# Open-Finance-Lab/RLSolver

Measured on AMD Instinct MI355X. Metric: env-steps/sec (all instances) on Gset G22 MaxCut; achieved HBM GB/s % peak, higher is better.
Workload: dtype u8

## Files before the change

rlsolver_amd/csrc/rls_step.hip:

```cpp
#include "rls_tile.h"
#include <cstdlib>

namespace rls {

constexpr int kStepPad = 128;

template <typename T> __device__ __forceinline__ T spin_flip(T v);
template <> __device__ __forceinline__ uint8_t spin_flip<uint8_t>(uint8_t v) { return v == 0 ? 1 : 0; }
template <> __device__ __forceinline__ float spin_flip<float>(float v) { return v == 0.0f ? 1.0f : 0.0f; }

template <typename T, bool WEIGHTED>
__device__ __forceinline__ int flip_gain(const T* row, int64_t a, const int32_t* __restrict__ rowptr,
                                         const int32_t* __restrict__ col, const int32_t* __restrict__ wgt,
                                         int lane) {
    const int r0 = rowptr[a], r1 = rowptr[a + 1];
    const bool xa = spin_is_set(row[a]);
    int acc = 0;
    for (int j = r0 + lane; j < r1; j += kWave) {
        const bool xn = spin_is_set(row[col[j]]);
        if constexpr (WEIGHTED) acc += (xn == xa) ? wgt[j] : -wgt[j];
        else acc += (xn != xa) ? 1 : 0;
    }
    if constexpr (WEIGHTED) {
        return wave_sum_i32(acc);
    } else {
        int c;
        if (r1 - r0 <= kWave) c = __popcll(ballot64(acc != 0));
        else c = wave_sum_i32(acc);
        return (r1 - r0) - 2 * c;
    }
}

template <bool NT, typename V> __device__ __forceinline__ V ld_vec(const V* p) {
    if constexpr (NT) return __builtin_nontemporal_load(p);
    else return *p;
}
enum : int { kStPlain = 0, kStNt = 1, kStWt = 2 };
template <int ST, typename V> __device__ __forceinline__ void st_vec(V* p, V v) {
    if constexpr (ST == kStNt) {
        __builtin_nontemporal_store(v, p);
    } else if constexpr (ST == kStWt) {
        static_assert(sizeof(V) == 16, "write-through stores are 16-byte vectors");
        asm volatile("global_store_dwordx4 %0, %1, off sc1\n\ts_nop 1" :: "v"(p), "v"(v) : "memory");
    } else {
        *p = v;
    }
}

__device__ __forceinline__ void wait_vmcnt_le(int k) {
    k = __builtin_amdgcn_readfirstlane(k);
#define RLS_W(n) case n: asm volatile("s_waitcnt vmcnt(" #n ")" ::: "memory"); break;
#define RLS_W8(b) RLS_W(b + 0) RLS_W(b + 1) RLS_W(b + 2) RLS_W(b + 3) RLS_W(b + 4) RLS_W(b + 5) RLS_W(b + 6) RLS_W(b + 7)
    switch (k) {
        case 0: asm volatile("s_waitcnt vmcnt(0)" ::: "memory"); break;
        RLS_W(1) RLS_W(2) RLS_W(3) RLS_W(4) RLS_W(5) RLS_W(6) RLS_W(7)
        RLS_W(8) RLS_W(9) RLS_W(10) RLS_W(11) RLS_W(12) RLS_W(13) RLS_W(14) RLS_W(15)
        RLS_W(16) RLS_W(17) RLS_W(18) RLS_W(19) RLS_W(20) RLS_W(21) RLS_W(22) RLS_W(23)
        RLS_W(24) RLS_W(25) RLS_W(26) RLS_W(27) RLS_W(28) RLS_W(29) RLS_W(30) RLS_W(31)
        RLS_W(32) RLS_W(33) RLS_W(34) RLS_W(35) RLS_W(36) RLS_W(37) RLS_W(38) RLS_W(39)
        RLS_W(40) RLS_W(41) RLS_W(42) RLS_W(43) RLS_W(44) RLS_W(45) RLS_W(46) RLS_W(47)
        RLS_W(48) RLS_W(49) RLS_W(50) RLS_W(51) RLS_W(52) RLS_W(53) RLS_W(54) RLS_W(55)
        RLS_W(56) RLS_W(57) RLS_W(58) RLS_W(59) RLS_W(60) RLS_W(61) RLS_W(62)
        default: asm volatile("s_waitcnt vmcnt(63)" ::: "memory"); break;
    }
#undef RLS_W8
#undef RLS_W
}

template <typename T, int EPW, int MODE, bool EMIT, bool VEC, bool WEIGHTED, bool NTL, int ST>
__global__ __launch_bounds__(256) void k_maxcut_step(const T* __restrict__ xin, T* __restrict__ xout,
                                                     int64_t B, int64_t N,
                                                     const int32_t* __restrict__ rowptr,
                                                     const int32_t* __restrict__ col,
                                                     const int32_t* __restrict__ wgt,
                                                     const int64_t* __restrict__ action,
                                                     int32_t* __restrict__ obj, float* __restrict__ reward,
                                                     float* __restrict__ cur, float* __restrict__ done,
                                                     float done_value, int align_lines) {
    extern __shared__ __attribute__((aligned(16))) unsigned char smem[];
    const int lane = threadIdx.x & (kWave - 1);
    const int wib = __builtin_amdgcn_readfirstlane((int)(threadIdx.x / kWave));
    using V = typename SpinVec<T>::type;
    constexpr int PER = SpinVec<T>::n;
    const int64_t wave_stride = (int64_t)gridDim.x * (blockDim.x / kWave);
  for (int64_t wave = (int64_t)blockIdx.x * (blockDim.x / kWave) + wib; wave * EPW < B; wave += wave_stride) {
    const int64_t b0 = wave * EPW;
    const int nenv = (int)((B - b0) < EPW ? (B - b0) : EPW);

    int64_t act[EPW];
#pragma unroll
    for (int k = 0; k < EPW; ++k) {
        const int64_t a = (k < nenv) ? action[b0 + k] : -1;
        act[k] = ((uint64_t)a < (uint64_t)N) ? a : -1;
    }

    int my_delta = 0;
    auto publish = [&]() {
        if (lane < nenv) {
            const int64_t b = b0 + lane;
            bool ok = false;
#pragma unroll
            for (int k = 0; k < EPW; ++k) if (lane == k) ok = act[k] >= 0;
            const int v = obj[b] + my_delta;
            obj[b] = v;
            reward[b] = ok ? (float)my_delta : __builtin_nanf("");
            if (cur) cur[b] = (float)v;
            if (done) done[b] = done_value;
        }
    };

    if constexpr (!EMIT) {
#pragma unroll
        for (int k = 0; k < EPW; ++k)
            if (act[k] >= 0) {
                const int d = flip_gain<T, WEIGHTED>(xin + (b0 + k) * N, act[k], rowptr, col, wgt, lane);
                if (lane == k) my_delta = d;
            }
        publish();
        if (lane < nenv) {
            int64_t a = -1;
#pragma unroll
            for (int k = 0; k < EPW; ++k) if (lane == k) a = act[k];
            if (a >= 0) {
                T* p = xout + (b0 + lane) * N + a;
                *p = spin_flip<T>(*p);
            }
        }
        return;
    } else if constexpr (!VEC) {
#pragma unroll
        for (int k = 0; k < EPW; ++k)
            if (act[k] >= 0) {
                const int d = flip_gain<T, WEIGHTED>(xin + (b0 + k) * N, act[k], rowptr, col, wgt, lane);
                if (lane == k) my_delta = d;
            }
        publish();
        const T* src = xin + b0 * N;
        T* dst = xout + b0 * N;
        const int64_t nel = (int64_t)nenv * N;
        for (int64_t i = lane; i < nel; i += kWave) {
            T v = src[i];
#pragma unroll
            for (int k = 0; k < EPW; ++k)
                if (act[k] >= 0 && i == (int64_t)k * N + act[k]) v = spin_flip<T>(v);
            dst[i] = v;
        }
        continue;
    } else {
        const V* src = reinterpret_cast<const V*>(xin + b0 * N);
        V* dst = reinterpret_cast<V*>(xout + b0 * N);
        const int64_t nel = (int64_t)nenv * N;
        const int64_t nvec = nel / PER;
        auto tail_copy = [&]() {
            for (int64_t i = nvec * PER + lane; i < nel; i += kWave) {
                T v = xin[b0 * N + i];
#pragma unroll
                for (int k = 0; k < EPW; ++k)
                    if (act[k] >= 0 && i == (int64_t)k * N + act[k]) v = spin_flip<T>(v);
                xout[b0 * N + i] = v;
            }
        };
        int64_t fvec[EPW];
        int fidx[EPW];
#pragma unroll
        for (int k = 0; k < EPW; ++k) {
            const int64_t rel = (act[k] < 0) ? -1 : (int64_t)k * N + act[k];
            fvec[k] = rel < 0 ? -1 : rel / PER;
            fidx[k] = (int)(rel < 0 ? 0 : rel % PER);
        }

        if constexpr (MODE == 0) {
#pragma unroll
            for (int k = 0; k < EPW; ++k)
                if (act[k] >= 0) {
                    const int d = flip_gain<T, WEIGHTED>(xin + (b0 + k) * N, act[k], rowptr, col, wgt, lane);
                    if (lane == k) my_delta = d;
                }
            publish();
#pragma unroll 4
            for (int64_t i = lane; i < nvec; i += kWave) {
                V v = ld_vec<NTL>(src + i);
#pragma unroll
                for (int k = 0; k < EPW; ++k)
                    if (i == fvec[k]) v = SpinVec<T>::flip_at(v, fidx[k]);
                st_vec<ST>(dst + i, v);
            }
            tail_copy();
        } else if constexpr (MODE == 1) {
            constexpr int BATCH = 8;
            V buf[BATCH];
            bool first = true;
            for (int64_t base = 0; base < nvec; base += BATCH * kWave) {
#pragma unroll
                for (int q = 0; q < BATCH; ++q) {
                    const int64_t i = base + q * kWave + lane;
                    if (i < nvec) buf[q] = ld_vec<NTL>(src + i);
                }
                if (first) {
                    first = false;
#pragma unroll
                    for (int k = 0; k < EPW; ++k)
                        if (act[k] >= 0) {
                            const int d = flip_gain<T, WEIGHTED>(xin + (b0 + k) * N, act[k], rowptr, col, wgt, lane);
                            if (lane == k) my_delta = d;
                        }
                    publish();
                }
#pragma unroll
                for (int q = 0; q < BATCH; ++q) {
                    const int64_t i = base + q * kWave + lane;
                    if (i < nvec) {
                        V v = buf[q];
#pragma unroll
                        for (int k = 0; k < EPW; ++k)
                            if (i == fvec[k]) v = SpinVec<T>::flip_at(v, fidx[k]);
                        st_vec<ST>(dst + i, v);
                    }
                }
            }
            tail_copy();
        } else if constexpr (MODE == 3) {
            unsigned char* region = smem + (size_t)wib * ((size_t)EPW * N * sizeof(T) + kStepPad);
            const int h_in = (int)((reinterpret_cast<uintptr_t>(src) >> 4) & 7), h_out = (int)((reinterpret_cast<uintptr_t>(dst) >> 4) & 7);
            const int h = (align_lines && h_in == h_out) ? h_in : 0;
            V* region_v = reinterpret_cast<V*>(region);
            V* stage_v = region_v + h;
            T* stage = reinterpret_cast<T*>(stage_v);
            const int nch = (int)((nvec + h + kWave - 1) / kWave);
            for (int64_t slot0 = 0; slot0 < nvec + h; slot0 += kWave) {
                const int64_t i = slot0 + lane - h;
                if (i >= 0 && i < nvec) glds16<NTL>(src + i, region_v + slot0);
            }
            if (nvec * PER < nel) {
                for (int64_t i = nvec * PER + lane; i < nel; i += kWave) stage[i] = xin[b0 * N + i];
                asm volatile("s_waitcnt vmcnt(0)" ::: "memory");
            }
            int r0[EPW], deg[EPW], nb[EPW], nlo = 0;
#pragma unroll
            for (int k = 0; k < EPW; ++k) {
                r0[k] = 0; deg[k] = 0; nb[k] = 0;
                if (act[k] >= 0) {
                    r0[k] = rowptr[act[k]];
                    deg[k] = rowptr[act[k] + 1] - r0[k];
                    if (deg[k] > 0) {
                        const int32_t* pn = col + r0[k] + (lane < deg[k] ? lane : 0);
                        asm volatile("global_load_dword %0, %1, off" : "=v"(nb[k]) : "v"(pn) : "memory");
                        ++nlo;
                    }
                }
            }
            const int keep = nch - 1 + nlo;
            for (int j = 0; j < nch; ++j) {
                wait_vmcnt_le(keep);
                const int64_t i = (int64_t)j * kWave + lane - h;
                if (i >= 0 && i < nvec) {
                    V v = stage_v[i];
#pragma unroll
                    for (int k = 0; k < EPW; ++k)
                        if (i == fvec[k]) v = SpinVec<T>::flip_at(v, fidx[k]);
                    st_vec<ST>(dst + i, v);
                }
            }
            tail_copy();
            wait_vmcnt_le(nch < 62 ? nch : 62);
#pragma unroll
            for (int k = 0; k < EPW; ++k) asm volatile("" : "+v"(nb[k]) :: "memory");
#pragma unroll
            for (int k = 0; k < EPW; ++k)
                if (act[k] >= 0) {
                    const T* row = stage + (int64_t)k * N;
                    const bool xa = spin_is_set(row[act[k]]);
                    int d;
                    if (deg[k] <= kWave) {
                        const bool on = lane < deg[k];
                        const bool xn = on ? spin_is_set(row[nb[k]]) : xa;
                        d = deg[k] - 2 * __popcll(ballot64(xn != xa));
                    } else {
                        d = flip_gain<T, WEIGHTED>(row, act[k], rowptr, col, wgt, lane);
                    }
                    if (lane == k) my_delta = d;
                }
            publish();
        } else {
            unsigned char* region = smem + (size_t)wib * ((size_t)EPW * N * sizeof(T) + kStepPad);
            const int h_in = align_lines ? (int)((reinterpret_cast<uintptr_t>(src) >> 4) & 7) : 0;
            const int h_out = align_lines ? (int)((reinterpret_cast<uintptr_t>(dst) >> 4) & 7) : 0;
            V* region_v = reinterpret_cast<V*>(region);
            V* stage_v = region_v + h_in;
            T* stage = reinterpret_cast<T*>(stage_v);
            for (int64_t slot0 = 0; slot0 < nvec + h_in; slot0 += kWave) {
                const int64_t i = slot0 + lane - h_in;
                if (i >= 0 && i < nvec) glds16<NTL>(src + i, region_v + slot0);
            }
            for (int64_t i = nvec * PER + lane; i < nel; i += kWave) stage[i] = xin[b0 * N + i];
            int r0[EPW], deg[EPW], nb[EPW], wv[EPW];
#pragma unroll
            for (int k = 0; k < EPW; ++k) {
                r0[k] = 0; deg[k] = 0; nb[k] = 0; wv[k] = 0;
                if (act[k] >= 0) {
                    r0[k] = rowptr[act[k]];
                    deg[k] = rowptr[act[k] + 1] - r0[k];
                    if (lane < deg[k]) {
                        nb[k] = col[r0[k] + lane];
                        if constexpr (WEIGHTED) wv[k] = wgt[r0[k] + lane];
                    }
                }
            }
            asm volatile("s_waitcnt vmcnt(0) lgkmcnt(0)" ::: "memory");
            __builtin_amdgcn_wave_barrier();
#pragma unroll
            for (int k = 0; k < EPW; ++k)
                if (act[k] >= 0) {
                    const T* row = stage + (int64_t)k * N;
                    const bool xa = spin_is_set(row[act[k]]);
                    int d;
                    if (deg[k] <= kWave) {
                        const bool on = lane < deg[k];
                        const bool xn = on ? spin_is_set(row[nb[k]]) : xa;
                        if constexpr (WEIGHTED) d = wave_sum_i32(on ? ((xn == xa) ? wv[k] : -wv[k]) : 0);
                        else d = deg[k] - 2 * __popcll(ballot64(xn != xa));
                    } else {
                        d = flip_gain<T, WEIGHTED>(row, act[k], rowptr, col, wgt, lane);
                    }
                    if (lane == k) my_delta = d;
                }
            publish();
            __builtin_amdgcn_wave_barrier();
            if (lane < nenv) {
                int64_t a = -1;
#pragma unroll
                for (int k = 0; k < EPW; ++k) if (lane == k) a = act[k];
                if (a >= 0) {
                    T* p = stage + (int64_t)lane * N + a;
                    *p = spin_flip<T>(*p);
                }
            }
            asm volatile("s_waitcnt lgkmcnt(0)" ::: "memory");
            __builtin_amdgcn_wave_barrier();
#pragma unroll 4
            for (int64_t slot0 = 0; slot0 < nvec + h_out; slot0 += kWave) {
                const int64_t i = slot0 + lane - h_out;
                if (i >= 0 && i < nvec) st_vec<ST>(dst + i, stage_v[i]);
            }
            for (int64_t i = nvec * PER + lane; i < nel; i += kWave) xout[b0 * N + i] = stage[i];
        }
    }
  }
}

struct StepKnobs { int nts, epw, wpb, persist, chase, align, wt; };
static StepKnobs step_knobs() {
    return StepKnobs{(int)knob(KN_STEP_NTS, -1), (int)knob(KN_STEP_EPW, 0), (int)knob(KN_STEP_WPB, 0), (int)knob(KN_STEP_PERSIST, -1),
                     (int)knob(KN_STEP_CHASE, -1), (int)knob(KN_STEP_ALIGN, 1), (int)knob(KN_STEP_WT, -1)};
}

}

using namespace rls;

extern "C" int rls_maxcut_step(const rls_graph* g, const void* x_in, void* x_out, int spin_bytes, int64_t B,
                               const int64_t* action, int32_t* obj, float* reward, float* cur, float* done,
                               float done_value, void* stream) {
    if (int rc = check_graph(g)) return rc;
    RLS_REQUIRE(B >= 0, RLS_EINVAL, "B < 0");
    if (B == 0) return RLS_OK;
    RLS_REQUIRE(x_in && x_out && action && obj && reward, RLS_EINVAL, "x_in/x_out/action/obj/reward is NULL");
    RLS_REQUIRE(spin_bytes == 1 || spin_bytes == 4, RLS_EINVAL, "spin_bytes must be 1 or 4");
    RLS_REQUIRE(!g->wgt, RLS_EUNSUPPORTED, "rls_maxcut_step counts cut edges (env_PPO.py:108-121): build the graph without weights");
    const int64_t N = g->num_nodes;
    const bool emit = (x_in != x_out);
    RLS_REQUIRE(!emit || (const char*)x_in + (size_t)B * N * spin_bytes <= (const char*)x_out ||
                    (const char*)x_out + (size_t)B * N * spin_bytes <= (const char*)x_in,
                RLS_EINVAL, "x_in and x_out overlap partially");
    const StepKnobs knobs = step_knobs();
    int epw_auto = 8;
    while (epw_auto > 1 && (int64_t)epw_auto * N * spin_bytes > 8192) epw_auto >>= 1;
    while (epw_auto < 8 && ((int64_t)epw_auto * N * spin_bytes) % 16 != 0) epw_auto <<= 1;
    const int epw = knobs.epw ? knobs.epw : (emit ? epw_auto : 4);
    const bool vec = ((((uintptr_t)x_in) | ((uintptr_t)x_out)) & 15) == 0 && ((int64_t)epw * N * spin_bytes) % 16 == 0;
    const size_t run_bytes = (size_t)epw * N * spin_bytes;
    int waves_per_block = knobs.wpb ? knobs.wpb : 4;
    if (!knobs.wpb && emit && vec && !knob_on(KN_STEP_NOSTAGE))
        while (waves_per_block > 1 && (size_t)waves_per_block * (run_bytes + kStepPad) > (size_t)kLdsBytes / 2) waves_per_block >>= 1;
    hipStream_t s = as_stream(stream);
    const bool lone_run = !knobs.wpb && emit && vec && waves_per_block == 1 && 2 * (run_bytes + kStepPad) > (size_t)kLdsBytes;
    if (lone_run) waves_per_block = 4;
    const bool staged = emit && vec && !lone_run && (size_t)waves_per_block * (run_bytes + kStepPad) <= (size_t)kLdsBytes &&
                        !knob_on(KN_STEP_NOSTAGE);
    const size_t lds = staged ? (size_t)waves_per_block * (run_bytes + kStepPad) : 0;
    int64_t nblocks = ceil_div(ceil_div(B, epw), waves_per_block);
    if (staged && knobs.persist != 0) {
        const int64_t per_cu = (int64_t)((size_t)kLdsBytes / lds) < 8 ? (int64_t)((size_t)kLdsBytes / lds) : 8;
        const int64_t resident = (int64_t)num_cus() * per_cu;
        const bool want = knobs.persist > 0 || (knobs.persist < 0 && false);
        if (want && nblocks > resident) nblocks = resident;
    }
    const dim3 grid((unsigned)nblocks), block(waves_per_block * kWave);
    const int64_t nch_run = ceil_div((int64_t)run_bytes, 16 * kWave);
    const bool chase = staged && nch_run + 1 + epw <= 62 && (knobs.chase > 0 || (knobs.chase < 0 && spin_bytes == 4));
    const bool nts = knobs.nts >= 0 ? knobs.nts != 0 : ((size_t)B * N * spin_bytes > ((size_t)256 << 20));
    const bool wt = !nts && (knobs.wt > 0 || (knobs.wt < 0 && !chase));

#define LAUNCH_STEP_E(T, EPW, MODE, EMIT, VEC, NTL, ST)                                                        \
    do {                                                                                                       \
        auto kern = k_maxcut_step<T, EPW, MODE, EMIT, VEC, false, NTL, ST>;                                    \
        if (lds > 64 * 1024)                                                                                   \
            ensure_dyn_lds((const void*)kern, lds); \
        hipLaunchKernelGGL(kern, grid, block, lds, s, (const T*)x_in, (T*)x_out, B, N, g->rowptr, g->col, g->wgt, \
                           action, obj, reward, cur, done, done_value, knobs.align);                           \
    } while (0)
#define LAUNCH_STEP(T, MODE, EMIT, VEC, NTL, ST)                            \
    do {                                                                    \
        if (epw == 2) LAUNCH_STEP_E(T, 2, MODE, EMIT, VEC, NTL, ST);        \
        else if (epw == 8) LAUNCH_STEP_E(T, 8, MODE, EMIT, VEC, NTL, ST);   \
        else if (epw == 1) LAUNCH_STEP_E(T, 1, MODE, EMIT, VEC, NTL, ST);   \
        else LAUNCH_STEP_E(T, 4, MODE, EMIT, VEC, NTL, ST);                 \
    } while (0)
#define DISPATCH_T(T)                                                                       \
    do {                                                                                    \
        if (!emit) LAUNCH_STEP_E(T, 4, 0, false, false, false, kStPlain);                   \
        else if (!vec) LAUNCH_STEP(T, 0, true, false, false, kStPlain);                     \
        else if (!staged) LAUNCH_STEP(T, 1, true, true, false, kStNt);                      \
        else if (chase && nts) LAUNCH_STEP(T, 3, true, true, true, kStNt);                  \
        else if (chase && wt) LAUNCH_STEP(T, 3, true, true, true, kStWt);                   \
        else if (chase) LAUNCH_STEP(T, 3, true, true, true, kStPlain);                      \
        else if (nts) LAUNCH_STEP(T, 2, true, true, true, kStNt);                           \
        else if (wt) LAUNCH_STEP(T, 2, true, true, true, kStWt);                            \
        else LAUNCH_STEP(T, 2, true, true, true, kStPlain);                                 \
    } while (0)
    RLS_REQUIRE(emit || epw == 4, RLS_EINVAL, "the in-place step runs 4 envs per wave");
    if (spin_bytes == 1) DISPATCH_T(uint8_t);
    else DISPATCH_T(float);
#undef DISPATCH_T
#undef LAUNCH_STEP
#undef LAUNCH_STEP_E
    return check_launch("k_maxcut_step");
}
```

Baseline: 1.556 billion.

## Overlap obj and neighbor loads with staging in MODE 2 step path

In the staged MODE 2 path, the objective value and neighbor column indices are now issued as early asynchronous global loads using inline asm, with a single vmcnt wait. Action bounds checks and rowptr reads move into scalar registers after the LDS staging loads are issued. Gain computation is restructured to use ballot popcount for all envs, with a fallback for high-degree nodes. Partial waves take the unstaged copy path, and the tail copy and publish are reordered after the stores. The aim is to hide load latency behind the bulk copy, at the cost of restricting MODE 2 to unweighted graphs and dropping the tail-element staging copy.

```diff
diff --git a/rlsolver_amd/csrc/rls_step.hip b/rlsolver_amd/csrc/rls_step.hip
--- a/rlsolver_amd/csrc/rls_step.hip
+++ b/rlsolver_amd/csrc/rls_step.hip
@@ -89,19 +89,27 @@
 
     int64_t act[EPW];
 #pragma unroll
-    for (int k = 0; k < EPW; ++k) {
-        const int64_t a = (k < nenv) ? action[b0 + k] : -1;
-        act[k] = ((uint64_t)a < (uint64_t)N) ? a : -1;
-    }
+    for (int k = 0; k < EPW; ++k) act[k] = (k < nenv) ? action[b0 + k] : -1;
+    auto check_actions = [&]() {
+#pragma unroll
+        for (int k = 0; k < EPW; ++k) act[k] = ((uint64_t)act[k] < (uint64_t)N) ? act[k] : -1;
+    };
+    if constexpr (!(EMIT && VEC && MODE == 2)) check_actions();
+
+    int obj_early = 0;
+    auto request_obj = [&]() {
+        const int32_t* po = obj + b0 + (lane < nenv ? lane : 0);
+        asm volatile("global_load_dword %0, %1, off" : "=v"(obj_early) : "v"(po) : "memory");
+    };
 
     int my_delta = 0;
-    auto publish = [&]() {
+    auto publish = [&](bool early = false) {
         if (lane < nenv) {
             const int64_t b = b0 + lane;
             bool ok = false;
 #pragma unroll
             for (int k = 0; k < EPW; ++k) if (lane == k) ok = act[k] >= 0;
-            const int v = obj[b] + my_delta;
+            const int v = (early ? obj_early : obj[b]) + my_delta;
             obj[b] = v;
             reward[b] = ok ? (float)my_delta : __builtin_nanf("");
             if (cur) cur[b] = (float)v;
@@ -162,14 +170,18 @@
         };
         int64_t fvec[EPW];
         int fidx[EPW];
-#pragma unroll
-        for (int k = 0; k < EPW; ++k) {
-            const int64_t rel = (act[k] < 0) ? -1 : (int64_t)k * N + act[k];
-            fvec[k] = rel < 0 ? -1 : rel / PER;
-            fidx[k] = (int)(rel < 0 ? 0 : rel % PER);
-        }
-
-        if constexpr (MODE == 0) {
+        auto set_flip_sites = [&]() {
+#pragma unroll
+            for (int k = 0; k < EPW; ++k) {
+                const int64_t rel = (act[k] < 0) ? -1 : (int64_t)k * N + act[k];
+                fvec[k] = rel < 0 ? -1 : rel / PER;
+                fidx[k] = (int)(rel < 0 ? 0 : rel % PER);
+            }
+        };
+        if constexpr (MODE == 1 || MODE == 3) set_flip_sites();
+
+        auto copy_unstaged = [&]() {
+            set_flip_sites();
 #pragma unroll
             for (int k = 0; k < EPW; ++k)
                 if (act[k] >= 0) {
@@ -186,6 +198,10 @@
                 st_vec<ST>(dst + i, v);
             }
             tail_copy();
+        };
+
+        if constexpr (MODE == 0) {
+            copy_unstaged();
         } else if constexpr (MODE == 1) {
             constexpr int BATCH = 8;
             V buf[BATCH];
@@ -220,6 +236,7 @@
             }
             tail_copy();
         } else if constexpr (MODE == 3) {
+            request_obj();
             unsigned char* region = smem + (size_t)wib * ((size_t)EPW * N * sizeof(T) + kStepPad);
             const int h_in = (int)((reinterpret_cast<uintptr_t>(src) >> 4) & 7), h_out = (int)((reinterpret_cast<uintptr_t>(dst) >> 4) & 7);
             const int h = (align_lines && h_in == h_out) ? h_in : 0;
@@ -265,6 +282,7 @@
             wait_vmcnt_le(nch < 62 ? nch : 62);
 #pragma unroll
             for (int k = 0; k < EPW; ++k) asm volatile("" : "+v"(nb[k]) :: "memory");
+            asm volatile("" : "+v"(obj_early) :: "memory");
 #pragma unroll
             for (int k = 0; k < EPW; ++k)
                 if (act[k] >= 0) {
@@ -280,8 +298,15 @@
                     }
                     if (lane == k) my_delta = d;
                 }
-            publish();
+            publish(true);
         } else {
+            static_assert(!WEIGHTED, "the staged gain counts cut edges");
+            if (nenv < EPW) {
+                check_actions();
+                copy_unstaged();
+                continue;
+            }
+            request_obj();
             unsigned char* region = smem + (size_t)wib * ((size_t)EPW * N * sizeof(T) + kStepPad);
             const int h_in = align_lines ? (int)((reinterpret_cast<uintptr_t>(src) >> 4) & 7) : 0;
             const int h_out = align_lines ? (int)((reinterpret_cast<uintptr_t>(dst) >> 4) & 7) : 0;
@@ -292,57 +317,66 @@
                 const int64_t i = slot0 + lane - h_in;
                 if (i >= 0 && i < nvec) glds16<NTL>(src + i, region_v + slot0);
             }
-            for (int64_t i = nvec * PER + lane; i < nel; i += kWave) stage[i] = xin[b0 * N + i];
-            int r0[EPW], deg[EPW], nb[EPW], wv[EPW];
-#pragma unroll
-            for (int k = 0; k < EPW; ++k) {
-                r0[k] = 0; deg[k] = 0; nb[k] = 0; wv[k] = 0;
-                if (act[k] >= 0) {
-                    r0[k] = rowptr[act[k]];
-                    deg[k] = rowptr[act[k] + 1] - r0[k];
-                    if (lane < deg[k]) {
-                        nb[k] = col[r0[k] + lane];
-                        if constexpr (WEIGHTED) wv[k] = wgt[r0[k] + lane];
+#pragma unroll
+            for (int k = 0; k < EPW; ++k) asm volatile("" : "+s"(act[k]));
+            check_actions();
+            int64_t ac[EPW];
+            int r0[EPW], r1[EPW], deg[EPW], nb[EPW];
+#pragma unroll
+            for (int k = 0; k < EPW; ++k) {
+                ac[k] = act[k] < 0 ? 0 : act[k];
+                r0[k] = rowptr[ac[k]];
+                r1[k] = rowptr[ac[k] + 1];
+            }
+#pragma unroll
+            for (int k = 0; k < EPW; ++k) {
+                asm volatile("" : "+s"(r0[k]), "+s"(r1[k]));
+                deg[k] = act[k] < 0 ? 0 : r1[k] - r0[k];
+            }
+#pragma unroll
+            for (int k = 0; k < EPW; ++k) {
+                nb[k] = 0;
+                if (deg[k] > 0) {
+                    const int32_t* pn = col + r0[k] + (lane < deg[k] ? lane : 0);
+                    asm volatile("global_load_dword %0, %1, off" : "=v"(nb[k]) : "v"(pn) : "memory");
+                }
+            }
+            asm volatile("s_waitcnt vmcnt(0)" : "+v"(obj_early) :: "memory");
+#pragma unroll
+            for (int k = 0; k < EPW; ++k) asm volatile("" : "+v"(nb[k]) :: "memory");
+            __builtin_amdgcn_wave_barrier();
+            T xa[EPW], xn[EPW];
+#pragma unroll
+            for (int k = 0; k < EPW; ++k) xa[k] = stage[(int64_t)k * N + ac[k]];
+#pragma unroll
+            for (int k = 0; k < EPW; ++k) xn[k] = stage[(int64_t)k * N + (lane < deg[k] ? (int64_t)nb[k] : ac[k])];
+            bool big = false;
+#pragma unroll
+            for (int k = 0; k < EPW; ++k) {
+                const bool cut = lane < deg[k] && spin_is_set(xn[k]) != spin_is_set(xa[k]);
+                const int d = deg[k] - 2 * __popcll(ballot64(cut));
+                if (lane == k) my_delta = d;
+                big = big || deg[k] > kWave;
+            }
+            if (big) {
+#pragma unroll
+                for (int k = 0; k < EPW; ++k)
+                    if (deg[k] > kWave) {
+                        const int d = flip_gain<T, WEIGHTED>(stage + (int64_t)k * N, act[k], rowptr, col, wgt, lane);
+                        if (lane == k) my_delta = d;
                     }
-                }
-            }
-            asm volatile("s_waitcnt vmcnt(0) lgkmcnt(0)" ::: "memory");
+            }
             __builtin_amdgcn_wave_barrier();
 #pragma unroll
             for (int k = 0; k < EPW; ++k)
-                if (act[k] >= 0) {
-                    const T* row = stage + (int64_t)k * N;
-                    const bool xa = spin_is_set(row[act[k]]);
-                    int d;
-                    if (deg[k] <= kWave) {
-                        const bool on = lane < deg[k];
-                        const bool xn = on ? spin_is_set(row[nb[k]]) : xa;
-                        if constexpr (WEIGHTED) d = wave_sum_i32(on ? ((xn == xa) ? wv[k] : -wv[k]) : 0);
-                        else d = deg[k] - 2 * __popcll(ballot64(xn != xa));
-                    } else {
-                        d = flip_gain<T, WEIGHTED>(row, act[k], rowptr, col, wgt, lane);
-                    }
-                    if (lane == k) my_delta = d;
-                }
-            publish();
-            __builtin_amdgcn_wave_barrier();
-            if (lane < nenv) {
-                int64_t a = -1;
-#pragma unroll
-                for (int k = 0; k < EPW; ++k) if (lane == k) a = act[k];
-                if (a >= 0) {
-                    T* p = stage + (int64_t)lane * N + a;
-                    *p = spin_flip<T>(*p);
-                }
-            }
-            asm volatile("s_waitcnt lgkmcnt(0)" ::: "memory");
+                if (lane == k && act[k] >= 0) stage[(int64_t)k * N + ac[k]] = spin_flip<T>(xa[k]);
             __builtin_amdgcn_wave_barrier();
 #pragma unroll 4
             for (int64_t slot0 = 0; slot0 < nvec + h_out; slot0 += kWave) {
                 const int64_t i = slot0 + lane - h_out;
                 if (i >= 0 && i < nvec) st_vec<ST>(dst + i, stage_v[i]);
             }
-            for (int64_t i = nvec * PER + lane; i < nel; i += kWave) xout[b0 * N + i] = stage[i];
+            publish(true);
         }
     }
   }
```

Measured after the change: 1.642 billion (median of 6 runs). +5.6%, better.

## Add LDS-staged u8 MODE 2 path overlapping operand loads with state copy

Applied to the files above, without the earlier changes.

Adds a specialized MODE 2 path for u8 spins with write-through stores. It stages the env rows into LDS via async global-to-LDS loads and issues the obj, neighbor and weight loads up front so they overlap with the row copy. Low-degree actions compute their gain with a single wave gather and a ballot popcount, and the flip is applied in LDS before the rows are stored back. This removes the serialized dependent loads of the generic path, but costs more LDS per wave and relies on hand-placed waitcnt and inline asm for correctness.

```diff
diff --git a/rlsolver_amd/csrc/rls_step.hip b/rlsolver_amd/csrc/rls_step.hip
--- a/rlsolver_amd/csrc/rls_step.hip
+++ b/rlsolver_amd/csrc/rls_step.hip
@@ -95,6 +95,19 @@
     }
 
     int my_delta = 0;
+    auto publish_from = [&](int obj_old) {
+        if (lane < nenv) {
+            const int64_t b = b0 + lane;
+            bool ok = false;
+#pragma unroll
+            for (int k = 0; k < EPW; ++k) if (lane == k) ok = act[k] >= 0;
+            const int v = obj_old + my_delta;
+            obj[b] = v;
+            reward[b] = ok ? (float)my_delta : __builtin_nanf("");
+            if (cur) cur[b] = (float)v;
+            if (done) done[b] = done_value;
+        }
+    };
     auto publish = [&]() {
         if (lane < nenv) {
             const int64_t b = b0 + lane;
@@ -219,6 +232,99 @@
                 }
             }
             tail_copy();
+        } else if constexpr (MODE == 2 && ST == kStWt && sizeof(T) == 1) {
+            unsigned char* region = smem + (size_t)wib * ((size_t)EPW * N * sizeof(T) + kStepPad);
+            const int h_src = (int)((reinterpret_cast<uintptr_t>(src) >> 4) & 7), h_dst = (int)((reinterpret_cast<uintptr_t>(dst) >> 4) & 7);
+            const int h_in = align_lines ? h_src : 0, h_out = align_lines ? h_dst : 0;
+            V* region_v = reinterpret_cast<V*>(region);
+            V* stage_v = region_v + h_in;
+            T* stage = reinterpret_cast<T*>(stage_v);
+            int obj_old;
+            {
+                const int32_t* po = obj + b0 + (lane < nenv ? lane : 0);
+                asm volatile("global_load_dword %0, %1, off" : "=v"(obj_old) : "v"(po) : "memory");
+            }
+            for (int64_t slot0 = 0; slot0 < nvec + h_in; slot0 += kWave) {
+                const int64_t i = slot0 + lane - h_in;
+                if (i >= 0 && i < nvec) glds16<NTL>(src + i, region_v + slot0);
+            }
+            int r0[EPW], deg[EPW], nb[EPW], wv[EPW];
+#pragma unroll
+            for (int k = 0; k < EPW; ++k) {
+                const int64_t ai = act[k] < 0 ? 0 : act[k];
+                r0[k] = rowptr[ai];
+                deg[k] = rowptr[ai + 1];
+            }
+            __builtin_amdgcn_sched_barrier(0);
+#pragma unroll
+            for (int k = 0; k < EPW; ++k) deg[k] -= r0[k];
+#pragma unroll
+            for (int k = 0; k < EPW; ++k) {
+                nb[k] = 0; wv[k] = 0;
+                if (act[k] >= 0 && deg[k] > 0) {
+                    const int32_t* pn = col + r0[k] + (lane < deg[k] ? lane : 0);
+                    asm volatile("global_load_dword %0, %1, off" : "=v"(nb[k]) : "v"(pn) : "memory");
+                    if constexpr (WEIGHTED) {
+                        const int32_t* pw = wgt + r0[k] + (lane < deg[k] ? lane : 0);
+                        asm volatile("global_load_dword %0, %1, off" : "=v"(wv[k]) : "v"(pw) : "memory");
+                    }
+                }
+            }
+            if (nvec * PER < nel) {
+                for (int64_t i = nvec * PER + lane; i < nel; i += kWave) stage[i] = xin[b0 * N + i];
+                asm volatile("s_waitcnt vmcnt(0)" ::: "memory");
+            }
+            auto operands_landed = [&]() {
+                asm volatile("" : "+v"(obj_old) :: "memory");
+#pragma unroll
+                for (int k = 0; k < EPW; ++k) {
+                    asm volatile("" : "+v"(nb[k]) :: "memory");
+                    if constexpr (WEIGHTED) asm volatile("" : "+v"(wv[k]) :: "memory");
+                }
+            };
+            auto gather = [&]() {
+#pragma unroll
+                for (int k = 0; k < EPW; ++k)
+                    if (act[k] >= 0) {
+                        const T* row = stage + (int64_t)k * N;
+                        const bool xa = spin_is_set(row[act[k]]);
+                        int d;
+                        if (deg[k] <= kWave) {
+                            const bool on = lane < deg[k];
+                            const bool xn = on ? spin_is_set(row[nb[k]]) : xa;
+                            if constexpr (WEIGHTED) d = wave_sum_i32(on ? ((xn == xa) ? wv[k] : -wv[k]) : 0);
+                            else d = deg[k] - 2 * __popcll(ballot64(xn != xa));
+                        } else {
+                            d = flip_gain<T, WEIGHTED>(row, act[k], rowptr, col, wgt, lane);
+                        }
+                        if (lane == k) my_delta = d;
+                    }
+            };
+            asm volatile("s_waitcnt vmcnt(0) lgkmcnt(0)" ::: "memory");
+            __builtin_amdgcn_wave_barrier();
+            operands_landed();
+            gather();
+            publish_from(obj_old);
+            __builtin_amdgcn_wave_barrier();
+            if (lane < nenv) {
+                int64_t a = -1;
+#pragma unroll
+                for (int k = 0; k < EPW; ++k) if (lane == k) a = act[k];
+                if (a >= 0) {
+                    T* p = stage + (int64_t)lane * N + a;
+                    *p = spin_flip<T>(*p);
+                }
+            }
+            asm volatile("s_waitcnt lgkmcnt(0)" ::: "memory");
+            __builtin_amdgcn_wave_barrier();
+#pragma unroll 4
+            for (int64_t slot0 = 0; slot0 < nvec + h_out; slot0 += kWave) {
+                const int64_t i = slot0 + lane - h_out;
+                if (i >= 0 && i < nvec) st_vec<ST>(dst + i, stage_v[i]);
+            }
+            for (int64_t i = nvec * PER + lane; i < nel; i += kWave) xout[b0 * N + i] = stage[i];
+            asm volatile("s_waitcnt lgkmcnt(0)" ::: "memory");
+            __builtin_amdgcn_wave_barrier();
         } else if constexpr (MODE == 3) {
             unsigned char* region = smem + (size_t)wib * ((size_t)EPW * N * sizeof(T) + kStepPad);
             const int h_in = (int)((reinterpret_cast<uintptr_t>(src) >> 4) & 7), h_out = (int)((reinterpret_cast<uintptr_t>(dst) >> 4) & 7);
```

Result: faster. 1.553 billion before, 1.628 billion after (median of 6 runs) (+4.8%).
